# neeharperi/FutureDet

Measured on AMD Instinct MI355X. Metric: sweeps/sec end-to-end (300k pts, 10-sweep voxel), higher is better.
Workload: dtype f32

## Files before the change

futuredet_amd/csrc/fd_spconv_c32.hip:

```cpp
#include "fd_spconv_chunk.h"

namespace {

namespace sk = fd::skeleton;
typedef float f32x16 __attribute__((ext_vector_type(16)));
typedef unsigned u32x4 __attribute__((ext_vector_type(4)));
constexpr int TM = 128, COUT = 32, TS = 4, WR = 1;
constexpr sk::Layout L = sk::layout(TM, COUT, TS, 32);
static_assert(((sk::kMaxTaps + TS - 1) / TS) * (TM / WR / 32) <= L.item_slot, "item list slot");

template <int CIN, int DEPTH, bool PLAN, bool SWZ>
__global__ void __launch_bounds__(256) spconv_f32_c32(const float *__restrict__ in, const float4 *__restrict__ wp, const float *__restrict__ bias,
                                                      const float *__restrict__ residual, int relu, const int *__restrict__ nbr, int64_t nbr_stride,
                                                      int K, int n_out, const int *__restrict__ n_out_dev, float *__restrict__ out, unsigned in_bytes,
                                                      const int *__restrict__ ranges, int rows_per_range) {
    constexpr int NCH = CIN / 8;
    constexpr int kPad = sk::pad_entry(TM);
    extern __shared__ __attribute__((aligned(16))) unsigned char smem[];
    int *s_list = reinterpret_cast<int *>(smem + L.list);
    unsigned short *s_items = reinterpret_cast<unsigned short *>(smem + L.items);
    unsigned char *s_cnt = smem + L.cnt;
    int *s_pad = reinterpret_cast<int *>(smem + L.pad);
    float *s_acc = reinterpret_cast<float *>(smem + L.acc);

    const int tid = threadIdx.x, lane = tid & 63, wave = __builtin_amdgcn_readfirstlane(tid >> 6);
    int r_begin, r_end, n_chunks, chunk_rows;
    sk::resolve_range(n_out, n_out_dev, ranges, rows_per_range, r_begin, r_end);
    if (r_begin >= r_end) return;
    sk::cut_chunks<TM>(r_begin, r_end, n_chunks, chunk_rows);
    int pre[sk::kSliceRegs<TM>];
    const int k_fetch = PLAN ? sk::kPlanRows : K;
    sk::fetch_slice<TM>(pre, nbr, nbr_stride, k_fetch, r_begin);

    const int ln = lane & 31, lh = lane >> 5;
    const int ts = wave, wr = 0;
    unsigned char *acc_bytes = reinterpret_cast<unsigned char *>(s_acc + ts * L.acc_copy);
    const __amdgpu_buffer_rsrc_t rsrc = __builtin_amdgcn_make_buffer_rsrc(const_cast<float *>(in), 0, (int)in_bytes, 0x00020000);
    unsigned short *items = s_items + wave * L.item_slot;

    for (int chunk = 0; chunk < n_chunks; ++chunk) {
        int row0, n_rows;
        if (!sk::chunk_span(r_begin, r_end, chunk_rows, chunk, row0, n_rows)) break;
        if constexpr (PLAN) {
            sk::stage_plan_chunk<TM, COUT, TS, 32>(pre, s_list, s_cnt, s_pad, s_acc, bias, residual, relu, row0, n_rows);
        } else {
            sk::stage_chunk<TM, COUT, TS, 32>(pre, s_list, s_pad, s_acc, bias, residual, relu, K, row0, n_rows);
            __syncthreads();
            sk::compact_taps<TM, WR>(s_list, s_cnt, K);
        }
        __syncthreads();
        if (chunk + 1 < n_chunks) sk::fetch_slice<TM>(pre, nbr, nbr_stride, k_fetch, row0 + chunk_rows);
        const int n_items = sk::build_items<TS, 32>(s_cnt, items, K, ts, wr);

        int k_r[DEPTH], row_r[DEPTH];
        u32x4 a_r[DEPTH][NCH];
        auto stage_a0 = [&](int it) -> int { return sk::stage_a0(items, n_items, it); };
        auto stage_a1 = [&](int it, int code_v, int &kk, int &e) { sk::stage_a1<TM, WR, 32>(s_list, s_pad, n_items, wr, ln, it, code_v, kk, e); };
        auto gather_offset = [&](int e) -> unsigned {
            const unsigned o = sk::entry_row_bytes<CIN>(e) + (unsigned)(lh * 16);
            return SWZ ? o ^ sk::entry_swz_bits(e) : o;
        };
        auto gather_step = [&](unsigned voff, int c) {
            return SWZ ? __builtin_amdgcn_raw_buffer_load_b128(rsrc, voff ^ (unsigned)(c * 32), 0, 0) : __builtin_amdgcn_raw_buffer_load_b128(rsrc, voff + c * 32, 0, 0);
        };
        float4 b[NCH];
        auto load_b = [&](int k) {
            const float4 *wk = wp + (int64_t)k * NCH * 64 + lane;
#pragma unroll
            for (int c = 0; c < NCH; ++c) b[c] = wk[c * 64];
        };
        int k_s, e_s, code_s;
#pragma unroll
        for (int d = 0; d < DEPTH - 1; ++d) {
            stage_a1(d, stage_a0(d), k_s, e_s);
            const unsigned vo = gather_offset(e_s);
#pragma unroll
            for (int c = 0; c < NCH; ++c) a_r[d][c] = gather_step(vo, c);
            k_r[d] = k_s;
            row_r[d] = e_s;
        }
        k_r[DEPTH - 1] = -1;
        row_r[DEPTH - 1] = kPad;
        stage_a1(DEPTH - 1, stage_a0(DEPTH - 1), k_s, e_s);
        code_s = stage_a0(DEPTH);
        if (n_items > 0) load_b(k_r[0]);

        for (int i0 = 0; i0 < n_items; i0 += DEPTH) {
#pragma unroll
            for (int d = 0; d < DEPTH; ++d) {
                const unsigned arow = sk::entry_local_row(row_r[d]);
                unsigned aoff[4];
#pragma unroll
                for (int q = 0; q < 4; ++q) aoff[q] = sk::acc_slot_bytes<COUT>(arow, (unsigned)(2 * q + lh));
                f32x16 acc;
#pragma unroll
                for (int q = 0; q < 4; ++q) {
                    const float4 v = *reinterpret_cast<const float4 *>(acc_bytes + aoff[q]);
                    acc[4 * q + 0] = v.x; acc[4 * q + 1] = v.y; acc[4 * q + 2] = v.z; acc[4 * q + 3] = v.w;
                }
                const int dn = (d + DEPTH - 1) % DEPTH;
                {
                    const int it = i0 + d + DEPTH - 1;
                    const unsigned vo = gather_offset(e_s);
                    k_r[dn] = k_s;
                    row_r[dn] = e_s;
#pragma unroll
                    for (int c = 0; c < NCH; ++c) a_r[dn][c] = gather_step(vo, c);
                    stage_a1(it + 1, code_s, k_s, e_s);
                    code_s = stage_a0(it + 2);
                }
                const int knext = k_r[(d + 1) % DEPTH];
                const bool reload = knext >= 0 && knext != k_r[d];
                __builtin_amdgcn_sched_barrier(0);
#pragma unroll
                for (int c = 0; c < NCH; ++c) {
                    const float4 av = __builtin_bit_cast(float4, a_r[d][c]);
                    acc = __builtin_amdgcn_mfma_f32_32x32x2f32(b[c].x, av.x, acc, 0, 0, 0);
                    acc = __builtin_amdgcn_mfma_f32_32x32x2f32(b[c].y, av.y, acc, 0, 0, 0);
                    acc = __builtin_amdgcn_mfma_f32_32x32x2f32(b[c].z, av.z, acc, 0, 0, 0);
                    acc = __builtin_amdgcn_mfma_f32_32x32x2f32(b[c].w, av.w, acc, 0, 0, 0);
                    if (reload) b[c] = (wp + (int64_t)knext * NCH * 64 + lane)[c * 64];
                }
#pragma unroll
                for (int q = 0; q < 4; ++q)
                    *reinterpret_cast<float4 *>(acc_bytes + aoff[q]) = make_float4(acc[4 * q + 0], acc[4 * q + 1], acc[4 * q + 2], acc[4 * q + 3]);
                __builtin_amdgcn_sched_barrier(0);
            }
        }
        __syncthreads();
        sk::epilogue<TM, COUT, TS>(s_acc, bias, residual, relu, out, row0, n_rows);
        __syncthreads();
    }
}

template <int CIN, int DEPTH, bool PLAN, bool SWZ>
int launch_c32(const fd::SpconvCall &c) {
    const unsigned in_bytes = (unsigned)(c.n_in * CIN * 4);
    int n_ranges = c.n_ranges, rows_per = 0;
    if (!c.ranges) sk::equal_rows_split(c.n_out, TM, c.n_out_dev != nullptr, n_ranges, rows_per);
    static std::atomic<uint64_t> lds_set{0};
    if (!fd::ensure_dynamic_lds(reinterpret_cast<const void *>(spconv_f32_c32<CIN, DEPTH, PLAN, SWZ>), (size_t)L.bytes, lds_set)) return 0;
    const void *wp = (const char *)c.wpacked + fd::spconv_weight_layout(c).c32.offset;
    hipLaunchKernelGGL((spconv_f32_c32<CIN, DEPTH, PLAN, SWZ>), dim3((unsigned)n_ranges), dim3(256), (size_t)L.bytes, c.stream, (const float *)c.in, (const float4 *)wp,
                       c.bias, (const float *)c.residual, sk::kernel_flags(c.relu, c.layout), PLAN ? c.plan : c.nbr, PLAN ? c.plan_stride : c.nbr_stride, c.K, c.n_out, c.n_out_dev, (float *)c.out, in_bytes, c.ranges, rows_per);
    return 1;
}

}

namespace fd {
int spconv_f32_c32_dispatch(const SpconvCall &c) {
    if (c.cout != 32 || c.cin != 32) return 0;
    if (!sk::entries_fit(c.n_in, c.cin)) return 0;
    if (c.layout & sk::kLayoutIn) return c.plan ? launch_c32<32, 3, true, true>(c) : launch_c32<32, 3, false, true>(c);
    return c.plan ? launch_c32<32, 3, true, false>(c) : launch_c32<32, 3, false, false>(c);
}
}
```

futuredet_amd/csrc/fd_spconv_chunk.h:

```cpp
#pragma once
#include "fd_common.h"

namespace fd {
namespace skeleton {

constexpr int kMaxTaps = 27;

constexpr int pad_entry(int tm) { return (int)(0xffffff00u | (unsigned)tm); }
__device__ __forceinline__ int pack_entry(int in_row, int local_row) { return (in_row << 8) | local_row; }
__device__ __forceinline__ unsigned entry_local_row(int e) { return (unsigned)e & 255u; }
template <int CIN>
__device__ __forceinline__ unsigned entry_row_bytes(int e) {
    static_assert(CIN == 16 || CIN == 32 || CIN == 64 || CIN == 128, "shift per CIN");
    const unsigned hi = (unsigned)e & 0xffffff00u;
    return CIN >= 64 ? hi << (CIN == 128 ? 1 : 0) : hi >> (CIN == 32 ? 1 : 2);
}

constexpr int kLayoutIn = 1, kLayoutResidual = 2, kLayoutOut = 4;
constexpr int kFlagRelu = 1, kFlagResidualSwz = kLayoutResidual, kFlagOutSwz = kLayoutOut;
constexpr int kernel_flags(int relu, int layout) { return (relu ? kFlagRelu : 0) | (layout & (kLayoutResidual | kLayoutOut)); }
__host__ __device__ constexpr unsigned swz_piece_bytes(unsigned s, unsigned r) { return (s ^ (r & 7u)) << 4; }
template <int COLS>
__device__ __forceinline__ int swz_col4(int c4, int row, bool on) {
    if constexpr (COLS < 32) return c4;
    return c4 ^ (row & (on ? 7 : 0));
}
__device__ __forceinline__ unsigned entry_swz_bits(int e) { return ((unsigned)e >> 4) & 0x70u; }

inline bool entries_fit(int64_t n_in_bound, int cin) { return n_in_bound < (1ll << 23) && n_in_bound * cin * 4 < (1ll << 31); }

struct Layout {
    int list;
    int items;
    int item_slot;
    int cnt;
    int pad;
    int acc;
    int acc_copy;
    int bytes;
};
constexpr int acc_copy_floats(int tm, int cout) { return (tm + 1) * cout; }
constexpr Layout layout(int tm, int cout, int ts, int item) {
    Layout l{};
    l.list = 0;
    l.items = l.list + (int)sizeof(int) * kMaxTaps * tm;
    l.item_slot = item == 16 ? kMaxTaps * (tm / 16) : 32;
    l.cnt = l.items + (int)sizeof(unsigned short) * 4 * l.item_slot;
    l.pad = l.cnt + 112;
    l.acc = l.pad + (int)sizeof(int) * item;
    l.acc_copy = acc_copy_floats(tm, cout);
    l.bytes = l.acc + (int)sizeof(float) * ts * l.acc_copy;
    return l;
}

template <int COUT>
__device__ __forceinline__ unsigned acc_swizzle(unsigned row) {
    static_assert(COUT == 16 || COUT == 32 || COUT == 64 || COUT == 128, "whole bank rows");
    constexpr int kSwzShift = COUT >= 64 ? 0 : COUT == 32 ? 1 : 2;
    constexpr unsigned kSwzMask = COUT >= 64 ? 15u : COUT == 32 ? 7u : 3u;
    return (row >> kSwzShift) & kSwzMask;
}
template <int COUT>
__device__ __forceinline__ int acc_slot(int row, int col) {
    return row * (COUT / 4) + (col ^ (int)acc_swizzle<COUT>((unsigned)row));
}
template <int COUT>
__device__ __forceinline__ unsigned acc_slot_bytes(unsigned row, unsigned col) {
    return row * (COUT * 4) + ((col ^ acc_swizzle<COUT>(row)) << 4);
}

__device__ __forceinline__ void resolve_range_of(int block, int n_blocks, int n_out, const int *n_out_dev, const int *ranges, int rows_per_range,
                                                 int &r_begin, int &r_end) {
    if (n_out_dev) n_out = fd::device_count(n_out, n_out_dev);
    if (ranges) {
        r_begin = ranges[block];
        r_end = ranges[block + 1];
    } else {
        if (n_out_dev) rows_per_range = (((n_out + n_blocks - 1) / n_blocks) + 15) & ~15;
        const int64_t b = (int64_t)block * rows_per_range;
        r_begin = (int)(b < n_out ? b : n_out);
        r_end = (int)(b + rows_per_range < n_out ? b + rows_per_range : n_out);
    }
    if (r_end > n_out) r_end = n_out;
}
__device__ __forceinline__ void resolve_range(int n_out, const int *n_out_dev, const int *ranges, int rows_per_range,
                                              int &r_begin, int &r_end) {
    resolve_range_of((int)blockIdx.x, (int)gridDim.x, n_out, n_out_dev, ranges, rows_per_range, r_begin, r_end);
}
template <int TM>
__device__ __forceinline__ void cut_chunks(int r_begin, int r_end, int &n_chunks, int &chunk_rows) {
    n_chunks = (r_end - r_begin + TM - 1) / TM;
    chunk_rows = (((r_end - r_begin + n_chunks - 1) / n_chunks) + 15) & ~15;
}
__device__ __forceinline__ bool chunk_span(int r_begin, int r_end, int chunk_rows, int chunk, int &row0, int &n_rows) {
    row0 = r_begin + chunk * chunk_rows;
    n_rows = (r_end - row0) < chunk_rows ? (r_end - row0) : chunk_rows;
    return n_rows > 0;
}
inline void equal_rows_split(int n_out, int tm, bool device_count, int &n_ranges, int &rows_per) {
    if (n_ranges <= 0) n_ranges = (n_out + tm - 1) / tm;
    rows_per = (((n_out + n_ranges - 1) / n_ranges) + 15) & ~15;
    if (!device_count) n_ranges = (n_out + rows_per - 1) / rows_per;
}

template <int TM>
constexpr int kSliceRegs = (kMaxTaps * TM + 255) / 256;

template <int TM>
__device__ __forceinline__ void fetch_slice(int (&pre)[kSliceRegs<TM>], const int *nbr, int64_t nbr_stride, int K, int row0) {
    const int tid = threadIdx.x;
#pragma unroll
    for (int i = 0; i < kSliceRegs<TM>; ++i) {
        const int t = tid + i * 256;
        int k = t / TM;
        const int r = t - k * TM;
        k = k < K ? k : K - 1;
        int64_t o = (int64_t)row0 + r;
        o = o < nbr_stride ? o : nbr_stride - 1;
        pre[i] = nbr[(int64_t)k * nbr_stride + o];
    }
}

template <int COUT>
constexpr bool kInitAcc = COUT <= 64;

template <int TM, int COUT, int TS>
__device__ __forceinline__ void init_acc(float *s_acc, const float *bias, const float *residual, int flags, int row0, int n_rows) {
    const int tid = threadIdx.x;
    if constexpr (kInitAcc<COUT>) {
        constexpr int C4i = COUT / 4, NINIT = TM * C4i / 256;
        static_assert(TM * C4i % 256 == 0, "whole passes");
        float4 iv[NINIT];
#pragma unroll
        for (int i = 0; i < NINIT; ++i) {
            const int t = tid + i * 256, c4 = t % C4i;
            iv[i] = bias ? reinterpret_cast<const float4 *>(bias)[c4] : make_float4(0.f, 0.f, 0.f, 0.f);
        }
        if (residual) {
            float4 rv[NINIT];
#pragma unroll
            for (int i = 0; i < NINIT; ++i) {
                const int t = tid + i * 256, r = t / C4i, c4 = t - r * C4i;
                const int rr = r < n_rows ? r : n_rows - 1;
                rv[i] = reinterpret_cast<const float4 *>(residual + (int64_t)(row0 + rr) * COUT)[swz_col4<COUT>(c4, row0 + rr, flags & kFlagResidualSwz)];
            }
#pragma unroll
            for (int i = 0; i < NINIT; ++i) { iv[i].x += rv[i].x; iv[i].y += rv[i].y; iv[i].z += rv[i].z; iv[i].w += rv[i].w; }
        }
#pragma unroll
        for (int i = 0; i < NINIT; ++i) {
            const int t = tid + i * 256, r = t / C4i, c4 = t - r * C4i;
            reinterpret_cast<float4 *>(s_acc)[acc_slot<COUT>(r, c4)] = r < n_rows ? iv[i] : make_float4(0.f, 0.f, 0.f, 0.f);
        }
        for (int t = TM * C4i + tid; t < TS * acc_copy_floats(TM, COUT) / 4; t += 256) reinterpret_cast<float4 *>(s_acc)[t] = make_float4(0.f, 0.f, 0.f, 0.f);
    } else {
        for (int t = tid; t < TS * acc_copy_floats(TM, COUT) / 4; t += 256) reinterpret_cast<float4 *>(s_acc)[t] = make_float4(0.f, 0.f, 0.f, 0.f);
    }
}

template <int TM, int COUT, int TS, int ITEM>
__device__ __forceinline__ void stage_chunk(const int (&pre)[kSliceRegs<TM>], int *s_list, int *s_pad, float *s_acc, const float *bias,
                                            const float *residual, int flags, int K, int row0, int n_rows) {
    const int tid = threadIdx.x;
    static_assert(256 % TM == 0, "a thread stages the same local row in every pass");
    const bool in_chunk = tid % TM < n_rows;
#pragma unroll
    for (int i = 0; i < kSliceRegs<TM>; ++i) {
        const int t = tid + i * 256;
        if (t < K * TM) s_list[t] = in_chunk ? pre[i] : -1;
    }
    init_acc<TM, COUT, TS>(s_acc, bias, residual, flags, row0, n_rows);
    if (tid < ITEM) s_pad[tid] = pad_entry(TM);
}

constexpr int kPlanRows = kMaxTaps + 1;
constexpr int kPlanTM = 128;
constexpr int kPlanCountWords = (kMaxTaps + 3) / 4;
inline int64_t plan_stride_for(int64_t n_out) { return (n_out + 8 + 63) / 64 * 64; }

template <int TM, int COUT, int TS, int ITEM>
__device__ __forceinline__ void stage_plan_chunk(const int (&pre)[kSliceRegs<TM>], int *s_list, unsigned char *s_cnt, int *s_pad, float *s_acc,
                                                 const float *bias, const float *residual, int flags, int row0, int n_rows) {
    const int tid = threadIdx.x;
    static_assert(TM == kPlanTM && 256 % TM == 0, "the plan is cut for 128-row chunks");
    static_assert(kSliceRegs<TM> * 256 >= kMaxTaps * TM + kPlanCountWords, "the count words ride in the slice's last register");
    const bool in_chunk = tid % TM < n_rows;
#pragma unroll
    for (int i = 0; i < kSliceRegs<TM>; ++i) {
        const int t = tid + i * 256;
        if (t < kMaxTaps * TM) {
            s_list[t] = in_chunk ? pre[i] : pad_entry(TM);
        } else if (t < kMaxTaps * TM + kPlanCountWords) {
            const int k0 = (t - kMaxTaps * TM) * 4;
#pragma unroll
            for (int q = 0; q < 4; ++q)
                if (k0 + q < kMaxTaps) s_cnt[(k0 + q) * 4] = (unsigned char)((unsigned)pre[i] >> (8 * q));
        }
    }
    init_acc<TM, COUT, TS>(s_acc, bias, residual, flags, row0, n_rows);
    if (tid < ITEM) s_pad[tid] = pad_entry(TM);
}

template <int TM, int WR>
__device__ __forceinline__ void compact_taps(int *s_list, unsigned char *s_cnt, int K) {
    const int lane = threadIdx.x & 63, wave = __builtin_amdgcn_readfirstlane(threadIdx.x >> 6);
    constexpr int RW = TM / WR, NH = (RW + 63) / 64;
    for (int k = wave; k < K; k += 4) {
#pragma unroll
        for (int wr = 0; wr < WR; ++wr) {
            const int base = k * TM + wr * RW;
            int count = 0;
            int v[NH];
#pragma unroll
            for (int h = 0; h < NH; ++h) {
                const int r = h * 64 + lane;
                v[h] = (r < RW) ? s_list[base + r] : -1;
            }
#pragma unroll
            for (int h = 0; h < NH; ++h) {
                const int r = h * 64 + lane;
                if (r < RW) s_list[base + r] = pad_entry(TM);
            }
#pragma unroll
            for (int h = 0; h < NH; ++h) {
                const int r = h * 64 + lane;
                const unsigned long long m = __ballot(v[h] >= 0);
                const int pos = count + __popcll(m & ((1ull << lane) - 1ull));
                if (v[h] >= 0) s_list[base + pos] = pack_entry(v[h], wr * RW + r);
                count += __popcll(m);
            }
            if (lane == 0) s_cnt[k * 4 + wr] = (unsigned char)count;
        }
    }
}

template <int TS, int ITEM>
__device__ __forceinline__ int build_items(const unsigned char *s_cnt, unsigned short *items, int K, int ts, int wr) {
    const int lane = threadIdx.x & 63;
    const int ng = (lane < K && (lane % TS) == ts) ? ((int)s_cnt[lane * 4 + wr] + ITEM - 1) / ITEM : 0;
    int inc = ng;
#pragma unroll
    for (int off = 1; off < 64; off <<= 1) {
        const int u = __shfl_up(inc, off);
        if (lane >= off) inc += u;
    }
    const int n_items = __builtin_amdgcn_readfirstlane(__shfl(inc, 63));
    for (int g = 0; g < ng; ++g) items[inc - ng + g] = (unsigned short)((lane << 3) | g);
    __builtin_amdgcn_fence(__ATOMIC_RELEASE, "workgroup");
    __builtin_amdgcn_wave_barrier();
    __builtin_amdgcn_fence(__ATOMIC_ACQUIRE, "workgroup");
    return n_items;
}

__device__ __forceinline__ int stage_a0(const unsigned short *items, int n_items, int it) { return (int)items[it < n_items ? it : 0]; }
template <int TM, int WR, int ITEM>
__device__ __forceinline__ void stage_a1(const int *s_list, const int *s_pad, int n_items, int wr, int lp, int it, int code_v, int &kk, int &e) {
    const bool v = it < n_items;
    const int code = __builtin_amdgcn_readfirstlane(code_v);
    const int ks = v ? (code >> 3) : 0;
    kk = v ? ks : -1;
    const int *lst = v ? s_list + ks * TM + wr * (TM / WR) + (code & 7) * ITEM : s_pad;
    e = lst[lp];
}

template <int TM, int COUT, int TS>
__device__ __forceinline__ void epilogue(float *s_acc, const float *bias, const float *residual, int flags,
                                         float *out, int row0, int n_rows) {
    const int tid = threadIdx.x;
    constexpr int C4 = COUT / 4;
    for (int t = tid; t < n_rows * C4; t += 256) {
        const int r = t / C4, c4 = t - r * C4;
        const int row = row0 + r;
        const int slot = acc_slot<COUT>(r, c4);
        float4 v = reinterpret_cast<const float4 *>(s_acc)[slot];
#pragma unroll
        for (int q = 1; q < TS; ++q) {
            const float4 v2 = reinterpret_cast<const float4 *>(s_acc + q * acc_copy_floats(TM, COUT))[slot];
            v.x += v2.x; v.y += v2.y; v.z += v2.z; v.w += v2.w;
        }
        if constexpr (!kInitAcc<COUT>) {
            if (bias) {
                const float4 bv = reinterpret_cast<const float4 *>(bias)[c4];
                v.x += bv.x; v.y += bv.y; v.z += bv.z; v.w += bv.w;
            }
            if (residual) {
                const float4 rv = reinterpret_cast<const float4 *>(residual + (int64_t)row * COUT)[swz_col4<COUT>(c4, row, flags & kFlagResidualSwz)];
                v.x += rv.x; v.y += rv.y; v.z += rv.z; v.w += rv.w;
            }
        }
        if (flags & kFlagRelu) { v.x = fmaxf(v.x, 0.f); v.y = fmaxf(v.y, 0.f); v.z = fmaxf(v.z, 0.f); v.w = fmaxf(v.w, 0.f); }
        reinterpret_cast<float4 *>(out + (int64_t)row * COUT)[swz_col4<COUT>(c4, row, flags & kFlagOutSwz)] = v;
    }
}

}
}
```

futuredet_amd/csrc/fd_spconv_v2.hip:

```cpp
#include "fd_spconv_chunk.h"

namespace {

namespace sk = fd::skeleton;
typedef float f32x4 __attribute__((ext_vector_type(4)));
typedef unsigned u32x4 __attribute__((ext_vector_type(4)));
typedef int i32x4 __attribute__((ext_vector_type(4)));

#ifdef FD_V2_TRACE
__device__ unsigned long long *g_trace;
#define FD_T(i)                                                                                  \
    do {                                                                                         \
        if (threadIdx.x == 0 && g_trace) g_trace[(size_t)blockIdx.x * 16 + (i)] = __builtin_readcyclecounter(); \
    } while (0)
#define FD_TV(i, v)                                                                    \
    do {                                                                               \
        if (threadIdx.x == 0 && g_trace) g_trace[(size_t)blockIdx.x * 16 + (i)] = (v); \
    } while (0)
#else
#define FD_T(i)
#define FD_TV(i, v)
#endif


constexpr int tap_splits(int cout) { return (cout == 32 || cout == 64) ? 2 : 1; }

template <int CIN, int COUT, int TM, int DEPTH, bool PLAN, bool SWZ>
__global__ void __launch_bounds__(256) spconv_f32_compact(const float *__restrict__ in, const float4 *__restrict__ wp,
                                                          const float *__restrict__ bias, const float *__restrict__ residual, int relu,
                                                          const int *__restrict__ nbr, int64_t nbr_stride, int K, int n_out,
                                                          const int *__restrict__ n_out_dev, float *__restrict__ out, unsigned in_bytes,
                                                          const int *__restrict__ ranges, int rows_per_range) {
    constexpr int NB = COUT / 16, NC = CIN / 16;
    constexpr int WC = NB == 8 ? 4 : (NB >= 2 ? 2 : 1);
    constexpr int NBW = NB / WC;
    constexpr int TS = tap_splits(COUT);
    constexpr int WR = 4 / (WC * TS);
    constexpr int NACC = NBW;
    static_assert((TM == 128 || TM == 64) && TM / WR >= 16, "local row uses 8 bits (0..TM, TM = scratch row)");
    static_assert(!PLAN || (TM == sk::kPlanTM && WR == 1), "the chunk plan holds the lists of 128-row chunks with one row set");
    static_assert(!SWZ || CIN >= 32, "rows of fewer than 128 bytes are never bank-spread");
    constexpr int kPad = sk::pad_entry(TM);
    constexpr sk::Layout L = sk::layout(TM, COUT, TS, 16);
    extern __shared__ __attribute__((aligned(16))) unsigned char smem[];
    int *s_list = reinterpret_cast<int *>(smem + L.list);
    unsigned short *s_items = reinterpret_cast<unsigned short *>(smem + L.items);
    unsigned char *s_cnt = smem + L.cnt;
    int *s_pad = reinterpret_cast<int *>(smem + L.pad);
    float *s_acc = reinterpret_cast<float *>(smem + L.acc);

    const int tid = threadIdx.x, lane = tid & 63, wave = __builtin_amdgcn_readfirstlane(tid >> 6);
    int r_begin, r_end, n_chunks, chunk_rows;
    sk::resolve_range(n_out, n_out_dev, ranges, rows_per_range, r_begin, r_end);
    if (r_begin >= r_end) return;
    FD_T(0);
    sk::cut_chunks<TM>(r_begin, r_end, n_chunks, chunk_rows);
    int pre[sk::kSliceRegs<TM>];
    const int k_fetch = PLAN ? sk::kPlanRows : K;
    sk::fetch_slice<TM>(pre, nbr, nbr_stride, k_fetch, r_begin);

    const int lrow = lane & 15, lq = lane >> 4;
    const int wc = wave % WC, wr = TS == 1 ? wave / WC : 0, ts = TS == 1 ? 0 : wave / WC;
    const int cb = wc * NBW * 16;
    unsigned char *acc_bytes = reinterpret_cast<unsigned char *>(s_acc + ts * L.acc_copy);
    const unsigned slot0 = (unsigned)(cb >> 2) + (unsigned)lq;
    const __amdgpu_buffer_rsrc_t rsrc = __builtin_amdgcn_make_buffer_rsrc(const_cast<float *>(in), 0, (int)in_bytes, 0x00020000);
    unsigned short *items = s_items + wave * L.item_slot;

    for (int chunk = 0; chunk < n_chunks; ++chunk) {
    int row0, n_rows;
    if (!sk::chunk_span(r_begin, r_end, chunk_rows, chunk, row0, n_rows)) break;
    if constexpr (PLAN) {
        sk::stage_plan_chunk<TM, COUT, TS, 16>(pre, s_list, s_cnt, s_pad, s_acc, bias, residual, relu, row0, n_rows);
    } else {
        sk::stage_chunk<TM, COUT, TS, 16>(pre, s_list, s_pad, s_acc, bias, residual, relu, K, row0, n_rows);
        __syncthreads();
        if (chunk == 0) FD_T(1);
        sk::compact_taps<TM, WR>(s_list, s_cnt, K);
    }
    __syncthreads();
    if (chunk == 0) FD_T(2);
    if (chunk + 1 < n_chunks) sk::fetch_slice<TM>(pre, nbr, nbr_stride, k_fetch, row0 + chunk_rows);
    const int n_items = sk::build_items<TS, 16>(s_cnt, items, K, ts, wr);

    int k_r[DEPTH];
    int row_r[DEPTH];
    u32x4 a_r[DEPTH][NC];
    auto stage_a0 = [&](int it) -> int { return sk::stage_a0(items, n_items, it); };
    auto stage_a1 = [&](int it, int code_v, int &kk, int &e) { sk::stage_a1<TM, WR, 16>(s_list, s_pad, n_items, wr, lrow, it, code_v, kk, e); };
    auto gather_offset = [&](int e) -> unsigned {
        const unsigned o = sk::entry_row_bytes<CIN>(e) + (unsigned)(lq * 16);
        return SWZ ? o ^ sk::entry_swz_bits(e) : o;
    };
    auto gather_chunk = [&](unsigned voff, int c) {
        return SWZ ? __builtin_amdgcn_raw_buffer_load_b128(rsrc, (voff ^ (unsigned)((c & 1) * 64)) + (c >> 1) * 128, 0, 0)
                   : __builtin_amdgcn_raw_buffer_load_b128(rsrc, voff + c * 64, 0, 0);
    };
    auto load_b = [&](int k, float4(&dst)[NC][NBW]) {
        const float4 *wk = wp + ((int64_t)k * NC * NB + wc * NBW) * 64 + lane;
#pragma unroll
        for (int c = 0; c < NC; ++c)
#pragma unroll
            for (int nw = 0; nw < NBW; ++nw) dst[c][nw] = wk[(c * NB + nw) * 64];
    };
    float4 b[NC][NBW];
    static_assert(DEPTH >= 2, "the slot freed by the previous item is refilled during the current item's MFMAs");
    int k_s, e_s, code_s;
#pragma unroll
    for (int d = 0; d < DEPTH - 1; ++d) {
        stage_a1(d, stage_a0(d), k_s, e_s);
        const unsigned vo = gather_offset(e_s);
#pragma unroll
        for (int c = 0; c < NC; ++c) a_r[d][c] = gather_chunk(vo, c);
        k_r[d] = k_s;
        row_r[d] = e_s;
    }
    k_r[DEPTH - 1] = -1;
    row_r[DEPTH - 1] = kPad;
    stage_a1(DEPTH - 1, stage_a0(DEPTH - 1), k_s, e_s);
    code_s = stage_a0(DEPTH);
    if (n_items > 0) load_b(k_r[0], b);
    if (chunk == 0) { FD_T(3); FD_TV(8, (unsigned long long)n_items); FD_TV(9, (unsigned long long)n_chunks); FD_TV(10, (unsigned long long)n_rows);
                      FD_TV(11, (unsigned long long)__builtin_amdgcn_s_getreg(4 | (31 << 11))); FD_TV(12, (unsigned long long)__builtin_amdgcn_s_getreg(20 | (31 << 11))); }
    FD_TV(13, (unsigned long long)(g_trace ? g_trace[(size_t)blockIdx.x * 16 + 13] : 0) + (unsigned long long)n_items);

    auto mfma_chunk = [&](const u32x4 &a4, const float4(&bc)[NBW], f32x4(&acc)[NACC]) {
        const float4 av = __builtin_bit_cast(float4, a4);
#pragma unroll
        for (int nw = 0; nw < NBW; ++nw) acc[nw] = __builtin_amdgcn_mfma_f32_16x16x4f32(bc[nw].x, av.x, acc[nw], 0, 0, 0);
#pragma unroll
        for (int nw = 0; nw < NBW; ++nw) acc[nw] = __builtin_amdgcn_mfma_f32_16x16x4f32(bc[nw].y, av.y, acc[nw], 0, 0, 0);
#pragma unroll
        for (int nw = 0; nw < NBW; ++nw) acc[nw] = __builtin_amdgcn_mfma_f32_16x16x4f32(bc[nw].z, av.z, acc[nw], 0, 0, 0);
#pragma unroll
        for (int nw = 0; nw < NBW; ++nw) acc[nw] = __builtin_amdgcn_mfma_f32_16x16x4f32(bc[nw].w, av.w, acc[nw], 0, 0, 0);
    };

    for (int i0 = 0; i0 < n_items; i0 += DEPTH) {
#pragma unroll
        for (int d = 0; d < DEPTH; ++d) {
            const unsigned arow = sk::entry_local_row(row_r[d]);
            unsigned aoff[NBW];
#pragma unroll
            for (int nw = 0; nw < NBW; ++nw) aoff[nw] = sk::acc_slot_bytes<COUT>(arow, slot0 + 4u * nw);
            f32x4 acc[NACC];
#pragma unroll
            for (int nw = 0; nw < NBW; ++nw) acc[nw] = *reinterpret_cast<const f32x4 *>(acc_bytes + aoff[nw]);
            const int dn = (d + DEPTH - 1) % DEPTH;
            unsigned vo;
            {
                const int it = i0 + d + DEPTH - 1;
                vo = gather_offset(e_s);
                k_r[dn] = k_s;
                row_r[dn] = e_s;
                stage_a1(it + 1, code_s, k_s, e_s);
                code_s = stage_a0(it + 2);
            }
            const int knext = k_r[(d + 1) % DEPTH];
            const bool reload = knext >= 0 && knext != k_r[d];
            constexpr bool kSpread = NC * 4 * NBW >= 16;
            if constexpr (!kSpread) {
#pragma unroll
                for (int c = 0; c < NC; ++c) a_r[dn][c] = gather_chunk(vo, c);
            }
            __builtin_amdgcn_sched_barrier(0);
            if (reload) {
                const float4 *wk = wp + ((int64_t)knext * NC * NB + wc * NBW) * 64 + lane;
#pragma unroll
                for (int c = 0; c < NC; ++c) {
                    mfma_chunk(a_r[d][c], b[c], acc);
                    if constexpr (kSpread) a_r[dn][c] = gather_chunk(vo, c);
#pragma unroll
                    for (int nw = 0; nw < NBW; ++nw) b[c][nw] = wk[(c * NB + nw) * 64];
                    __builtin_amdgcn_sched_group_barrier(0x008, 4 * NBW, 0);
                    __builtin_amdgcn_sched_group_barrier(0x020, (kSpread ? 1 : 0) + NBW, 0);
                }
            } else {
#pragma unroll
                for (int c = 0; c < NC; ++c) {
                    mfma_chunk(a_r[d][c], b[c], acc);
                    if constexpr (kSpread) {
                        a_r[dn][c] = gather_chunk(vo, c);
                        __builtin_amdgcn_sched_group_barrier(0x008, 4 * NBW, 0);
                        __builtin_amdgcn_sched_group_barrier(0x020, 1, 0);
                    }
                }
            }
#pragma unroll
            for (int nw = 0; nw < NBW; ++nw) *reinterpret_cast<f32x4 *>(acc_bytes + aoff[nw]) = acc[nw];
            __builtin_amdgcn_sched_barrier(0);
        }
    }
    if (chunk == 0) FD_T(4);
    __syncthreads();
    if (chunk == 0) FD_T(5);
    sk::epilogue<TM, COUT, TS>(s_acc, bias, residual, relu, out, row0, n_rows);
    __syncthreads();
    if (chunk == 0) FD_T(6);
    }
    FD_T(7);
}

inline size_t lds_request(int cin, int cout, int tm) {
    const size_t lds = (size_t)sk::layout(tm, cout, tap_splits(cout), 16).bytes;
    return (cin == 64 && cout == 64 && tm == 128 && lds < 56 * 1024) ? (size_t)56 * 1024 : lds;
}

constexpr bool has_swz_gather(int cin, int cout, int tm) { return cin == cout && (cin == 64 || cin == 128) && tm == sk::kPlanTM; }

template <int CIN, int COUT, int TM, int DEPTH, bool PLAN = false, bool SWZ = false>
int launch_compact(const fd::SpconvCall &c) {
    if constexpr (!PLAN && !SWZ) {
        if ((c.layout & sk::kLayoutIn) && !has_swz_gather(CIN, COUT, TM)) return 0;
        if ((c.layout & (sk::kLayoutResidual | sk::kLayoutOut)) && COUT < 32) return 0;
        if constexpr (has_swz_gather(CIN, COUT, TM)) {
            if (c.layout & sk::kLayoutIn) return launch_compact<CIN, COUT, TM, DEPTH, false, true>(c);
        }
    }
    if constexpr (!PLAN && ((CIN == COUT && COUT >= 32) || COUT == 2 * CIN) && TM == sk::kPlanTM) {
        if (c.plan) return launch_compact<CIN, COUT, TM, DEPTH, true, SWZ>(c);
    }
    const size_t lds_req = lds_request(CIN, COUT, TM);
    static std::atomic<uint64_t> lds_set{0};
    auto kern = spconv_f32_compact<CIN, COUT, TM, DEPTH, PLAN, SWZ>;
    if (!fd::ensure_dynamic_lds(reinterpret_cast<const void *>(kern), lds_req, lds_set)) return 0;
    const unsigned in_bytes = (unsigned)(c.n_in * CIN * 4);
    int n_ranges = c.n_ranges, rows_per = 0;
    if (!c.ranges) sk::equal_rows_split(c.n_out, TM, c.n_out_dev != nullptr, n_ranges, rows_per);
    const void *wp = (const char *)c.wpacked + fd::spconv_weight_layout(c).base.offset;
    hipLaunchKernelGGL(kern, dim3((unsigned)n_ranges), dim3(256), lds_req, c.stream, (const float *)c.in, (const float4 *)wp, c.bias,
                       (const float *)c.residual, sk::kernel_flags(c.relu, c.layout), PLAN ? c.plan : c.nbr, PLAN ? c.plan_stride : c.nbr_stride, c.K, c.n_out, c.n_out_dev,
                       (float *)c.out, in_bytes, c.ranges, rows_per);
    return 1;
}

constexpr int kWorkRows = 8;
constexpr int kRowCost = 24;
__global__ void __launch_bounds__(256) block_work_kernel(const int *__restrict__ nbr, int64_t nbr_stride, int K, int n_out,
                                                         const int *__restrict__ n_out_dev, unsigned row_cost, unsigned *__restrict__ work) {
    n_out = fd::device_count(n_out, n_out_dev);
    const int n_blocks = (n_out + kWorkRows - 1) / kWorkRows;
    const int lane = threadIdx.x & 63;
    const int64_t wave = (int64_t)blockIdx.x * 4 + (threadIdx.x >> 6);
    const int64_t o = wave * 64 + lane;
    if (wave * 8 >= n_blocks) return;
    unsigned w = row_cost;
    for (int k = 0; k < K; ++k) {
        const bool v = o < n_out && nbr[(int64_t)k * nbr_stride + o] >= 0;
        const unsigned long long m = __ballot(v);
        const unsigned byte = (unsigned)(m >> (8 * (lane & 7))) & 0xffu;
        w += (unsigned)__popc(byte) * 2u + (byte ? 1u : 0u);
    }
    if (lane < 8 && wave * 8 + lane < n_blocks) work[wave * 8 + lane] = w;
}

__global__ void __launch_bounds__(1024) range_split_kernel(const unsigned *__restrict__ work, int n_out, const int *__restrict__ n_out_dev,
                                                           int n_ranges, int *__restrict__ ranges) {
    n_out = fd::device_count(n_out, n_out_dev);
    const int n_blocks = (n_out + kWorkRows - 1) / kWorkRows;
    __shared__ unsigned long long s_seg[16];
    __shared__ unsigned long long s_total;
    const int tid = threadIdx.x, lane = tid & 63, wave = tid >> 6;
    if (n_blocks == 0) {
        for (int j = tid; j <= n_ranges; j += 1024) ranges[j] = 0;
        return;
    }
    const int seg = (((n_blocks + 15) / 16) + 63) & ~63;
    const int b_lo = wave * seg, b_hi = min(n_blocks, b_lo + seg);
    constexpr int kU = 16;
    unsigned long long sum = 0;
    for (int c0 = b_lo; c0 < b_hi; c0 += 64 * kU) {
        unsigned wv[kU];
#pragma unroll
        for (int u = 0; u < kU; ++u) {
            const int bb = c0 + 64 * u + lane;
            wv[u] = work[bb < b_hi ? bb : b_hi - 1];
        }
#pragma unroll
        for (int u = 0; u < kU; ++u) sum += (c0 + 64 * u + lane < b_hi) ? wv[u] : 0u;
    }
#pragma unroll
    for (int o = 32; o > 0; o >>= 1) sum += __shfl_xor(sum, o);
    if (lane == 0) s_seg[wave] = sum;
    __syncthreads();
    if (tid == 0) {
        unsigned long long run = 0;
        for (int w = 0; w < 16; ++w) { const unsigned long long v = s_seg[w]; s_seg[w] = run; run += v; }
        s_total = run;
    }
    __syncthreads();
    const unsigned long long total = s_total > 0 ? s_total : 1ull;
    const double scale = (double)n_ranges / (2.0 * (double)total);
    auto range_of = [&](unsigned long long ex, unsigned w) -> int {
        const int r = (int)((double)(2ull * ex + w) * scale);
        return r < n_ranges ? r : n_ranges - 1;
    };
    unsigned long long run = s_seg[wave];
    int prev = -1;
    if (b_lo > 0 && b_lo < n_blocks) {
        const unsigned wp = work[b_lo - 1];
        prev = range_of(run - wp, wp);
    }
    constexpr int kB = 8;
    __shared__ unsigned s_buf[16][64 * (kB + 1)];
    unsigned *buf = s_buf[wave];
    for (int c0 = b_lo; c0 < b_hi; c0 += 64 * kB) {
#pragma unroll
        for (int u = 0; u < kB; ++u) {
            const int e = 64 * u + lane, bb = c0 + e;
            buf[(e / kB) * (kB + 1) + e % kB] = bb < b_hi ? work[bb] : 0u;
        }
        __builtin_amdgcn_fence(__ATOMIC_RELEASE, "workgroup");
        __builtin_amdgcn_wave_barrier();
        __builtin_amdgcn_fence(__ATOMIC_ACQUIRE, "workgroup");
        unsigned w[kB];
        unsigned tot = 0;
#pragma unroll
        for (int i = 0; i < kB; ++i) {
            w[i] = buf[lane * (kB + 1) + i];
            tot += w[i];
        }
        unsigned inc = tot;
#pragma unroll
        for (int o = 1; o < 64; o <<= 1) {
            const unsigned u = __shfl_up(inc, o);
            if (lane >= o) inc += u;
        }
        unsigned long long ex = run + (inc - tot);
        const int first = c0 + lane * kB;
        int last_rg = prev;
        {
            unsigned long long e2 = ex;
#pragma unroll
            for (int i = 0; i < kB; ++i) {
                if (first + i < b_hi) last_rg = range_of(e2, w[i]);
                e2 += w[i];
            }
        }
        int before = __shfl_up(last_rg, 1);
        if (lane == 0) before = prev;
        if (first >= b_hi) last_rg = before;
#pragma unroll
        for (int i = 0; i < kB; ++i) {
            const int bb = first + i;
            if (bb < b_hi) {
                const int rg = range_of(ex, w[i]);
                for (int j = before + 1; j <= rg; ++j) ranges[j] = bb * kWorkRows;
                before = rg;
                if (bb == n_blocks - 1)
                    for (int j = rg + 1; j <= n_ranges; ++j) ranges[j] = n_out;
            }
            ex += w[i];
        }
        const int n_valid = min(64 * kB, b_hi - c0);
        prev = __shfl(last_rg, (n_valid - 1) / kB);
        run += __shfl(inc, 63);
        __builtin_amdgcn_wave_barrier();
    }
}

constexpr int kPlanSplit = 4;
__global__ void __launch_bounds__(256) chunk_plan_kernel(const int *__restrict__ nbr, int64_t nbr_stride, int n_out, const int *__restrict__ n_out_dev,
                                                         const int *__restrict__ ranges, int rows_per_range, int *__restrict__ plan, int64_t plan_stride) {
    constexpr int TM = sk::kPlanTM, K = sk::kMaxTaps, NT = (K + 3) / 4, NH = TM / 64;
    constexpr int kPad = sk::pad_entry(TM);
    const int lane = threadIdx.x & 63, wave = __builtin_amdgcn_readfirstlane(threadIdx.x >> 6);
    int r_begin, r_end, n_chunks, chunk_rows;
    sk::resolve_range(n_out, n_out_dev, ranges, rows_per_range, r_begin, r_end);
    if (r_begin < 0 || r_begin >= r_end) return;
    sk::cut_chunks<TM>(r_begin, r_end, n_chunks, chunk_rows);
    for (int chunk = blockIdx.y; chunk < n_chunks; chunk += kPlanSplit) {
        int row0, n_rows;
        if (!sk::chunk_span(r_begin, r_end, chunk_rows, chunk, row0, n_rows)) break;
        int v[NT][NH];
#pragma unroll
        for (int j = 0; j < NT; ++j) {
            const int k = wave + 4 * j < K ? wave + 4 * j : K - 1;
#pragma unroll
            for (int h = 0; h < NH; ++h) {
                const int r = h * 64 + lane;
                const int rr = r < n_rows ? r : n_rows - 1;
                v[j][h] = nbr[(int64_t)k * nbr_stride + row0 + rr];
                if (r >= n_rows) v[j][h] = -1;
            }
        }
#pragma unroll
        for (int j = 0; j < NT; ++j) {
            const int k = wave + 4 * j;
            if (k >= K) break;
            int *list = plan + (int64_t)k * plan_stride + row0;
            int count = 0;
#pragma unroll
            for (int h = 0; h < NH; ++h) {
                const unsigned long long m = __ballot(v[j][h] >= 0);
                const int pos = count + __popcll(m & ((1ull << lane) - 1ull));
                if (v[j][h] >= 0) list[pos] = sk::pack_entry(v[j][h], h * 64 + lane);
                count += __popcll(m);
            }
#pragma unroll
            for (int h = 0; h < NH; ++h) {
                const int p = h * 64 + lane;
                if (p >= count && p < n_rows) list[p] = kPad;
            }
            if (lane == 0) reinterpret_cast<unsigned char *>(plan + (int64_t)K * plan_stride + row0)[k] = (unsigned char)count;
        }
    }
}

struct PlanSource {
    const unsigned long long *words;
    const int *prefix;
    const int *out_coords;
    const int *n_out_dev;
    const int *ranges;
    int *plan;
    int64_t plan_stride;
    fd::IndexGeom gi;
    int n_out, n_ranges, rows_per_range;
    int s[3], p[3];
};
constexpr int kMaxPlanSources = 8;
struct PlanSources {
    PlanSource t[kMaxPlanSources];
};

__device__ __forceinline__ int tap_row(unsigned long long w, int base, int iz, int D) {
    return (iz >= 0 && iz < D && ((w >> iz) & 1ull)) ? base + __popcll(w & ((1ull << iz) - 1ull)) : -1;
}

__global__ void __launch_bounds__(256) index_plan_kernel(const PlanSources S) {
    constexpr int TM = sk::kPlanTM, K = sk::kMaxTaps, NH = TM / 64, NCOL = 3;
    constexpr int kPad = sk::pad_entry(TM);
    const PlanSource &t = S.t[blockIdx.z];
    if ((int)blockIdx.x >= t.n_ranges) return;
    const int lane = threadIdx.x & 63, wave = __builtin_amdgcn_readfirstlane(threadIdx.x >> 6);
    int r_begin, r_end, n_chunks, chunk_rows;
    sk::resolve_range_of((int)blockIdx.x, t.n_ranges, t.n_out, t.n_out_dev, t.ranges, t.rows_per_range, r_begin, r_end);
    if (r_begin < 0 || r_begin >= r_end) return;
    sk::cut_chunks<TM>(r_begin, r_end, n_chunks, chunk_rows);
    const fd::IndexGeom gi = t.gi;
    for (int chunk = blockIdx.y; chunk < n_chunks; chunk += kPlanSplit) {
        int row0, n_rows;
        if (!sk::chunk_span(r_begin, r_end, chunk_rows, chunk, row0, n_rows)) break;
        int4 c[NH];
#pragma unroll
        for (int h = 0; h < NH; ++h) {
            const int r = h * 64 + lane;
            c[h] = reinterpret_cast<const int4 *>(t.out_coords)[row0 + (r < n_rows ? r : n_rows - 1)];
        }
        unsigned long long w[NCOL][NH];
        int base[NCOL][NH];
#pragma unroll
        for (int j = 0; j < NCOL; ++j) {
            const int c9 = wave + 4 * j, ky = c9 / 3, kx = c9 - 3 * ky;
#pragma unroll
            for (int h = 0; h < NH; ++h) {
                const int iy = c[h].z * t.s[1] - t.p[1] + ky;
                const int ix = c[h].w * t.s[2] - t.p[2] + kx;
                const bool ok = c9 < 9 && h * 64 + lane < n_rows && iy >= 0 && iy < gi.H && ix >= 0 && ix < gi.W;
                const int64_t col = ok ? fd::col_of(gi, c[h].x, iy, ix) : 0;
                const unsigned long long wv = t.words[col];
                base[j][h] = t.prefix[col];
                w[j][h] = ok ? wv : 0ull;
            }
        }
#pragma unroll
        for (int j = 0; j < NCOL; ++j) {
            const int c9 = wave + 4 * j;
            if (c9 >= 9) break;
            for (int kz = 0; kz < 3; ++kz) {
                const int k = kz * 9 + c9;
                int *list = t.plan + (int64_t)k * t.plan_stride + row0;
                int v[NH];
#pragma unroll
                for (int h = 0; h < NH; ++h) v[h] = tap_row(w[j][h], base[j][h], c[h].y * t.s[0] - t.p[0] + kz, gi.D);
                int count = 0;
// ... 193 lines not shown
```

Baseline: 290.9.

## Cut per-item address and index overhead in sparse conv inner loops

Weight loads now go through buffer resource descriptors with scalar per-tap offsets instead of 64-bit flat pointer arithmetic, in both the c32 and v2 kernels. In the c32 kernel, item codes are read once into a lane register and pulled out with readlane rather than reloaded from LDS each step. Accumulator slot addresses are computed as raw LDS addresses with XOR-based swizzle terms, which relies on the accumulator region being aligned to the swizzle span. The intent is fewer VALU and LDS instructions around the MFMA chain, at the cost of stricter alignment assumptions and a wider LDS layout.

Result: faster. 294.5, median of 6 (+1.3%).

```diff
diff --git a/futuredet_amd/csrc/fd_spconv_c32.hip b/futuredet_amd/csrc/fd_spconv_c32.hip
--- a/futuredet_amd/csrc/fd_spconv_c32.hip
+++ b/futuredet_amd/csrc/fd_spconv_c32.hip
@@ -5,6 +5,9 @@
 namespace sk = fd::skeleton;
 typedef float f32x16 __attribute__((ext_vector_type(16)));
 typedef unsigned u32x4 __attribute__((ext_vector_type(4)));
+typedef __attribute__((address_space(3))) unsigned char lds_u8;
+typedef float f32x4 __attribute__((ext_vector_type(4)));
+typedef __attribute__((address_space(3))) f32x4 lds_f4;
 constexpr int TM = 128, COUT = 32, TS = 4, WR = 1;
 constexpr sk::Layout L = sk::layout(TM, COUT, TS, 32);
 static_assert(((sk::kMaxTaps + TS - 1) / TS) * (TM / WR / 32) <= L.item_slot, "item list slot");
@@ -16,7 +19,7 @@
                                                       const int *__restrict__ ranges, int rows_per_range) {
     constexpr int NCH = CIN / 8;
     constexpr int kPad = sk::pad_entry(TM);
-    extern __shared__ __attribute__((aligned(16))) unsigned char smem[];
+    extern __shared__ __attribute__((aligned(256))) unsigned char smem[];
     int *s_list = reinterpret_cast<int *>(smem + L.list);
     unsigned short *s_items = reinterpret_cast<unsigned short *>(smem + L.items);
     unsigned char *s_cnt = smem + L.cnt;
@@ -34,8 +37,13 @@
 
     const int ln = lane & 31, lh = lane >> 5;
     const int ts = wave, wr = 0;
-    unsigned char *acc_bytes = reinterpret_cast<unsigned char *>(s_acc + ts * L.acc_copy);
+    static_assert(L.acc % sk::acc_span(COUT) == 0 && (L.acc_copy * 4) % sk::acc_span(COUT) == 0, "tile copies start at multiples of the swizzle span");
+    const unsigned tile_off = (unsigned)(__UINTPTR_TYPE__)(lds_u8 *)smem + (unsigned)(L.acc + ts * L.acc_copy * 4);
+    const unsigned acc_c0 = (unsigned)lh * 16u;
     const __amdgpu_buffer_rsrc_t rsrc = __builtin_amdgcn_make_buffer_rsrc(const_cast<float *>(in), 0, (int)in_bytes, 0x00020000);
+    constexpr int kTapBytes = NCH * 64 * 16;
+    const __amdgpu_buffer_rsrc_t wrsrc = __builtin_amdgcn_make_buffer_rsrc(const_cast<float4 *>(wp), 0, K * kTapBytes, 0x00020000);
+    const unsigned wlane = (unsigned)lane * 16u;
     unsigned short *items = s_items + wave * L.item_slot;
 
     for (int chunk = 0; chunk < n_chunks; ++chunk) {
@@ -51,11 +59,12 @@
         __syncthreads();
         if (chunk + 1 < n_chunks) sk::fetch_slice<TM>(pre, nbr, nbr_stride, k_fetch, row0 + chunk_rows);
         const int n_items = sk::build_items<TS, 32>(s_cnt, items, K, ts, wr);
+        const int codes = sk::item_codes<L.item_slot>(items);
 
         int k_r[DEPTH], row_r[DEPTH];
         u32x4 a_r[DEPTH][NCH];
-        auto stage_a0 = [&](int it) -> int { return sk::stage_a0(items, n_items, it); };
-        auto stage_a1 = [&](int it, int code_v, int &kk, int &e) { sk::stage_a1<TM, WR, 32>(s_list, s_pad, n_items, wr, ln, it, code_v, kk, e); };
+        auto stage_a0 = [&](int it) -> int { return sk::stage_a0_reg(codes, n_items, it); };
+        auto stage_a1 = [&](int it, int code, int &kk, int &e) { sk::stage_a1_s<TM, WR, 32>(s_list, s_pad, n_items, wr, ln, it, code, kk, e); };
         auto gather_offset = [&](int e) -> unsigned {
             const unsigned o = sk::entry_row_bytes<CIN>(e) + (unsigned)(lh * 16);
             return SWZ ? o ^ sk::entry_swz_bits(e) : o;
@@ -64,10 +73,12 @@
             return SWZ ? __builtin_amdgcn_raw_buffer_load_b128(rsrc, voff ^ (unsigned)(c * 32), 0, 0) : __builtin_amdgcn_raw_buffer_load_b128(rsrc, voff + c * 32, 0, 0);
         };
         float4 b[NCH];
+        auto load_b_step = [&](int k, int c) {
+            return __builtin_bit_cast(float4, __builtin_amdgcn_raw_buffer_load_b128(wrsrc, wlane, k * kTapBytes + c * 64 * 16, 0));
+        };
         auto load_b = [&](int k) {
-            const float4 *wk = wp + (int64_t)k * NCH * 64 + lane;
 #pragma unroll
-            for (int c = 0; c < NCH; ++c) b[c] = wk[c * 64];
+            for (int c = 0; c < NCH; ++c) b[c] = load_b_step(k, c);
         };
         int k_s, e_s, code_s;
 #pragma unroll
@@ -88,14 +99,14 @@
         for (int i0 = 0; i0 < n_items; i0 += DEPTH) {
 #pragma unroll
             for (int d = 0; d < DEPTH; ++d) {
-                const unsigned arow = sk::entry_local_row(row_r[d]);
+                const unsigned aterm = (tile_off + sk::acc_row_term<COUT>(sk::entry_local_row(row_r[d]))) ^ acc_c0;
                 unsigned aoff[4];
 #pragma unroll
-                for (int q = 0; q < 4; ++q) aoff[q] = sk::acc_slot_bytes<COUT>(arow, (unsigned)(2 * q + lh));
+                for (int q = 0; q < 4; ++q) aoff[q] = aterm ^ (unsigned)(q * 32);
                 f32x16 acc;
 #pragma unroll
                 for (int q = 0; q < 4; ++q) {
-                    const float4 v = *reinterpret_cast<const float4 *>(acc_bytes + aoff[q]);
+                    const f32x4 v = *reinterpret_cast<const lds_f4 *>((__UINTPTR_TYPE__)aoff[q]);
                     acc[4 * q + 0] = v.x; acc[4 * q + 1] = v.y; acc[4 * q + 2] = v.z; acc[4 * q + 3] = v.w;
                 }
                 const int dn = (d + DEPTH - 1) % DEPTH;
@@ -112,18 +123,32 @@
                 const int knext = k_r[(d + 1) % DEPTH];
                 const bool reload = knext >= 0 && knext != k_r[d];
                 __builtin_amdgcn_sched_barrier(0);
-#pragma unroll
-                for (int c = 0; c < NCH; ++c) {
+                auto mfma_step = [&](int c) {
                     const float4 av = __builtin_bit_cast(float4, a_r[d][c]);
                     acc = __builtin_amdgcn_mfma_f32_32x32x2f32(b[c].x, av.x, acc, 0, 0, 0);
                     acc = __builtin_amdgcn_mfma_f32_32x32x2f32(b[c].y, av.y, acc, 0, 0, 0);
                     acc = __builtin_amdgcn_mfma_f32_32x32x2f32(b[c].z, av.z, acc, 0, 0, 0);
                     acc = __builtin_amdgcn_mfma_f32_32x32x2f32(b[c].w, av.w, acc, 0, 0, 0);
-                    if (reload) b[c] = (wp + (int64_t)knext * NCH * 64 + lane)[c * 64];
+                };
+                auto write_back = [&]() {
+#pragma unroll
+                    for (int q = 0; q < 4; ++q)
+                        *reinterpret_cast<lds_f4 *>((__UINTPTR_TYPE__)aoff[q]) = f32x4{acc[4 * q + 0], acc[4 * q + 1], acc[4 * q + 2], acc[4 * q + 3]};
+                };
+                if (reload) {
+#pragma unroll
+                    for (int c = 0; c < NCH; ++c) {
+                        mfma_step(c);
+                        b[c] = load_b_step(knext, c);
+                    }
+                    write_back();
+                    asm volatile("; c32 item, reload copy");
+                } else {
+#pragma unroll
+                    for (int c = 0; c < NCH; ++c) mfma_step(c);
+                    write_back();
+                    asm volatile("; c32 item, plain copy");
                 }
-#pragma unroll
-                for (int q = 0; q < 4; ++q)
-                    *reinterpret_cast<float4 *>(acc_bytes + aoff[q]) = make_float4(acc[4 * q + 0], acc[4 * q + 1], acc[4 * q + 2], acc[4 * q + 3]);
                 __builtin_amdgcn_sched_barrier(0);
             }
         }
diff --git a/futuredet_amd/csrc/fd_spconv_chunk.h b/futuredet_amd/csrc/fd_spconv_chunk.h
--- a/futuredet_amd/csrc/fd_spconv_chunk.h
+++ b/futuredet_amd/csrc/fd_spconv_chunk.h
@@ -40,6 +40,7 @@
     int bytes;
 };
 constexpr int acc_copy_floats(int tm, int cout) { return (tm + 1) * cout; }
+constexpr int acc_span(int cout) { return cout >= 64 ? 256 : cout * 4; }
 constexpr Layout layout(int tm, int cout, int ts, int item) {
     Layout l{};
     l.list = 0;
@@ -48,6 +49,7 @@
     l.cnt = l.items + (int)sizeof(unsigned short) * 4 * l.item_slot;
     l.pad = l.cnt + 112;
     l.acc = l.pad + (int)sizeof(int) * item;
+    if (item == 32) l.acc = (l.acc + acc_span(cout) - 1) / acc_span(cout) * acc_span(cout);
     l.acc_copy = acc_copy_floats(tm, cout);
     l.bytes = l.acc + (int)sizeof(float) * ts * l.acc_copy;
     return l;
@@ -67,6 +69,11 @@
 template <int COUT>
 __device__ __forceinline__ unsigned acc_slot_bytes(unsigned row, unsigned col) {
     return row * (COUT * 4) + ((col ^ acc_swizzle<COUT>(row)) << 4);
+}
+
+template <int COUT>
+__device__ __forceinline__ unsigned acc_row_term(unsigned row) {
+    return row * (COUT * 4) + (acc_swizzle<COUT>(row) << 4);
 }
 
 __device__ __forceinline__ void resolve_range_of(int block, int n_blocks, int n_out, const int *n_out_dev, const int *ranges, int rows_per_range,
@@ -263,6 +270,21 @@
     e = lst[lp];
 }
 
+template <int SLOT>
+__device__ __forceinline__ int item_codes(const unsigned short *items) {
+    static_assert(SLOT <= 64 && (SLOT & (SLOT - 1)) == 0, "one code per lane");
+    return (int)items[threadIdx.x & (SLOT - 1)];
+}
+__device__ __forceinline__ int stage_a0_reg(int codes, int n_items, int it) { return __builtin_amdgcn_readlane(codes, it < n_items ? it : 0); }
+template <int TM, int WR, int ITEM>
+__device__ __forceinline__ void stage_a1_s(const int *s_list, const int *s_pad, int n_items, int wr, int lp, int it, int code, int &kk, int &e) {
+    const bool v = it < n_items;
+    const int ks = v ? (code >> 3) : 0;
+    kk = v ? ks : -1;
+    const int *lst = v ? s_list + ks * TM + wr * (TM / WR) + (code & 7) * ITEM : s_pad;
+    e = lst[lp];
+}
+
 template <int TM, int COUT, int TS>
 __device__ __forceinline__ void epilogue(float *s_acc, const float *bias, const float *residual, int flags,
                                          float *out, int row0, int n_rows) {
diff --git a/futuredet_amd/csrc/fd_spconv_v2.hip b/futuredet_amd/csrc/fd_spconv_v2.hip
--- a/futuredet_amd/csrc/fd_spconv_v2.hip
+++ b/futuredet_amd/csrc/fd_spconv_v2.hip
@@ -65,6 +65,9 @@
     unsigned char *acc_bytes = reinterpret_cast<unsigned char *>(s_acc + ts * L.acc_copy);
     const unsigned slot0 = (unsigned)(cb >> 2) + (unsigned)lq;
     const __amdgpu_buffer_rsrc_t rsrc = __builtin_amdgcn_make_buffer_rsrc(const_cast<float *>(in), 0, (int)in_bytes, 0x00020000);
+    constexpr int kTapBytes = NC * NB * 64 * 16;
+    const __amdgpu_buffer_rsrc_t wrsrc = __builtin_amdgcn_make_buffer_rsrc(const_cast<float4 *>(wp), 0, K * kTapBytes, 0x00020000);
+    const unsigned w_lane = (unsigned)(lane * 16 + wc * NBW * 64 * 16);
     unsigned short *items = s_items + wave * L.item_slot;
 
     for (int chunk = 0; chunk < n_chunks; ++chunk) {
@@ -96,12 +99,14 @@
         return SWZ ? __builtin_amdgcn_raw_buffer_load_b128(rsrc, (voff ^ (unsigned)((c & 1) * 64)) + (c >> 1) * 128, 0, 0)
                    : __builtin_amdgcn_raw_buffer_load_b128(rsrc, voff + c * 64, 0, 0);
     };
+    auto load_w = [&](int k, int c, int nw) {
+        return __builtin_bit_cast(float4, __builtin_amdgcn_raw_buffer_load_b128(wrsrc, w_lane, k * kTapBytes + (c * NB + nw) * 64 * 16, 0));
+    };
     auto load_b = [&](int k, float4(&dst)[NC][NBW]) {
-        const float4 *wk = wp + ((int64_t)k * NC * NB + wc * NBW) * 64 + lane;
 #pragma unroll
         for (int c = 0; c < NC; ++c)
 #pragma unroll
-            for (int nw = 0; nw < NBW; ++nw) dst[c][nw] = wk[(c * NB + nw) * 64];
+            for (int nw = 0; nw < NBW; ++nw) dst[c][nw] = load_w(k, c, nw);
     };
     float4 b[NC][NBW];
     static_assert(DEPTH >= 2, "the slot freed by the previous item is refilled during the current item's MFMAs");
@@ -165,13 +170,12 @@
             }
             __builtin_amdgcn_sched_barrier(0);
             if (reload) {
-                const float4 *wk = wp + ((int64_t)knext * NC * NB + wc * NBW) * 64 + lane;
 #pragma unroll
                 for (int c = 0; c < NC; ++c) {
                     mfma_chunk(a_r[d][c], b[c], acc);
                     if constexpr (kSpread) a_r[dn][c] = gather_chunk(vo, c);
 #pragma unroll
-                    for (int nw = 0; nw < NBW; ++nw) b[c][nw] = wk[(c * NB + nw) * 64];
+                    for (int nw = 0; nw < NBW; ++nw) b[c][nw] = load_w(knext, c, nw);
                     __builtin_amdgcn_sched_group_barrier(0x008, 4 * NBW, 0);
                     __builtin_amdgcn_sched_group_barrier(0x020, (kSpread ? 1 : 0) + NBW, 0);
                 }
```
